# cherise215/advchain

Measured on AMD Instinct MI355X. Metric: augmented images/sec (N adv steps, chain=noise+bias+morph+affine), higher is better.
Workload: dtype f32

## Files before the change

advchain_amd/_lib.py:

```python
import ctypes
import os
from ctypes import c_char_p, c_float, c_int, c_int64, c_void_p

_HERE = os.path.dirname(os.path.abspath(__file__))
LIB_PATH = os.path.join(_HERE, "csrc", "libadvchain_hip.so")

_P, _I, _L, _F = c_void_p, c_int, c_int64, c_float

PROTOTYPES = {
    "advchain_version": (_I, []),
    "advchain_last_error": (c_char_p, []),
    "advchain_set_deterministic": (None, [_I]),
    "advchain_get_deterministic": (_I, []),
    "advchain_grid_sample_fwd": (_I, [_P, _P, _P, _L, _L, _I, _P, _P, _I, _I, _I, _P]),
    "advchain_grid_sample_fwd_ride": (_I, [_P, _P, _P, _P, _P, _L, _L, _I, _P, _P, _I, _I, _I, _I, _P]),
    "advchain_scatter_workspace": (_L, [_L, _I, _P]),
    "advchain_grid_sample_bwd": (_I, [_P, _P, _P, _P, _P, _P, _L, _L, _I, _P, _P, _I, _I, _I, _I, _P]),
    "advchain_window_stage_workspace": (_L, [_L, _L, _I, _P]),
    "advchain_grid_sample_bwd_staged": (_I, [_P, _P, _P, _P, _P, _P, _L, _L, _I, _P, _P, _I, _I, _I, _I, _P, _P]),
    "advchain_last_bwd_route": (_I, []),
    "advchain_det_warp_workspace": (_L, [_L, _L, _I, _P]),
    "advchain_grid_sample_bwd_det": (_I, [_P, _P, _P, _P, _P, _P, _L, _L, _I, _P, _P, _I, _I, _I, _P]),
    "advchain_compose_self_fwd": (_I, [_P, _P, _P, _L, _I, _P, _I, _P, _P]),
    "advchain_compose_self_bwd": (_I, [_P, _P, _P, _P, _I, _I, _L, _I, _P, _P]),
    "advchain_affine_warp_fwd": (_I, [_P, _P, _P, _L, _L, _I, _P, _I, _I, _P]),
    "advchain_affine_warp_fwd_ride": (_I, [_P, _P, _P, _P, _P, _L, _L, _I, _P, _I, _I, _I, _P]),
    "advchain_affine_warp_bwd_workspace": (_L, [_L, _I, _P]),
    "advchain_affine_warp_bwd": (_I, [_P, _P, _P, _P, _P, _P, _L, _L, _I, _P, _I, _I, _P]),
    "advchain_affine_warp_bwd_det": (_I, [_P, _P, _P, _P, _P, _P, _P, _L, _L, _I, _P, _I, _I, _P]),
    "advchain_affine_theta_fwd": (_I, [_P, _P, _F, _P, _P, _L, _I, _P]),
    "advchain_affine_theta_bwd": (_I, [_P, _P, _F, _P, _P, _P, _L, _I, _P]),
    "advchain_tp_interp_fwd": (_I, [_P, _P, _P, _P, _P, _P, _P, _L, _L, _I, _I, _F, _P, _P, _P]),
    "advchain_tp_interp_fwd_smoothed_pair": (_I, [_P, _P, _P, _P, _P, _P, _P, _P, _L, _L, _I, _F, _P, _P, _F, _P]),
    "advchain_band_reduce_axis": (_I, [_P, _P, _P, _P, _P, _P, _P, _P, _I, _L, _L, _F, _P]),
    "advchain_band_reduce_rows_dense": (_I, [_P, _P, _P, _P, _P, _L, _L, _L, _L, _F, _P]),
    "advchain_bias_field_fwd": (_I, [_P, _P, _P, _P, _P, _P, _P, _P, _P, _L, _L, _F, _I, _F, _P]),
    "advchain_bias_field_bwd": (_I, [_P, _P, _P, _P, _P, _P, _P, _P, _P, _P, _L, _L, _F, _I, _F, _P]),
    "advchain_bias_rows_per_wg": (_I, [_P, _L]),
    "advchain_bias_field_fwd_rows": (_I, [_P, _P, _P, _P, _P, _P, _P, _P, _P, _L, _L, _F, _I, _F, _I, _P]),
    "advchain_bias_field_bwd_rows": (_I, [_P, _P, _P, _P, _P, _P, _P, _P, _P, _P, _L, _L, _F, _I, _F, _I, _P]),
    "advchain_bias_field_bwd_reduced": (_I, [_P, _P, _P, _P, _P, _P, _P, _P, _P, _P, _L, _L, _F, _I, _F, _P, _P, _L, _I, _P]),
    "advchain_gauss_axis": (_I, [_P, _P, _P, _L, _L, _I, _P, _I, _P, _I, _I, _F, _P]),
    "advchain_gauss_axis_generic": (_I, [_P, _P, _L, _I, _P, _I, _P, _I, _F, _P]),
    "advchain_max_displacement": (_I, [_P, _P, _L, _I, _P, _P]),
    "advchain_grid_sample_bicubic2d_fwd": (_I, [_P, _P, _P, _L, _L, _P, _P, _I, _P]),
    "advchain_grid_sample_bicubic2d_bwd": (_I, [_P, _P, _P, _P, _P, _L, _L, _P, _P, _I, _P]),
    "advchain_affine_grid2d_fwd": (_I, [_P, _P, _L, _P, _P]),
    "advchain_affine_grid2d_bwd_workspace": (_L, [_L, _P]),
    "advchain_affine_grid2d_bwd": (_I, [_P, _P, _P, _L, _P, _P]),
    "advchain_slot_rows_max": (_I, [_P, _P, _L, _L, _I, _P]),
    "advchain_demons_compose_pair_fwd": (_I, [_P, _P, _P, _P, _P, _P, _P, _P, _P, _P, _P, _P, _P, _L, _I, _I, _P, _P, _F, _F, _I, _P]),
    "advchain_demons_compose_pair_bwd": (_I, [_P, _P, _P, _P, _P, _P, _P, _P, _P, _P, _P, _P, _P, _P, _P, _P, _P, _L, _P, _P, _P, _L,
                                              _I, _I, _P, _F, _F, _P]),
    "advchain_bounds_check": (_I, [_P, _P, _P, _L, _P, _P]),
    "advchain_expo_chain_fused_levels": (_I, [_L, _I, _P, _I, _P]),
    "advchain_expo_chain_fwd": (_I, [_P, _P, _P, _L, _I, _P, _I, _P, _P, _P, _P]),
    "advchain_expo_chain_bwd": (_I, [_P, _P, _P, _P, _P, _P, _P, _L, _I, _P, _I, _P]),
    "advchain_gauss_xy": (_I, [_P, _P, _P, _L, _L, _I, _P, _P, _I, _I, _F, _P, _P, _L]),
    "advchain_gauss_small": (_I, [_P, _P, _L, _I, _P, _P, _I, _F, _P]),
    "advchain_gauss_small_pair": (_I, [_P, _P, _L, _I, _P, _P, _F, _I, _P]),
    "advchain_axpy": (_I, [_P, _P, _P, _F, _L, _P]),
    "advchain_sign_axpy": (_I, [_P, _P, _P, _F, _L, _P, _P, _P]),
    "advchain_nonzero_mask": (_I, [_P, _P, _L, _P]),
    "advchain_consistency_finish": (_I, [_P, _P, _P, _P, _I, _P]),
    "advchain_norm_workspace": (_L, [_L, _L]),
    "advchain_norm_axpy": (_I, [_P, _P, _P, _P, _F, _L, _L, _P]),
    "advchain_norm_axpy_gated": (_I, [_P, _P, _P, _P, _F, _L, _L, _P, _P, _P]),
    "advchain_update_multi": (_I, [_P, _I, _P, _P]),
    "advchain_consistency_fwd": (_I, [_P, _P, _P, _P, _P, _P, _P, _L, _L, _I, _P, _I, _I, _I, _I, _P]),
    "advchain_consistency_bwd": (_I, [_P, _P, _P, _P, _P, _P, _F, _F, _F, _F, _I, _L, _L, _I, _P, _I, _P]),
    "advchain_consistency_fused_fwd": (_I, [_P, _P, _P, _P, _P, _L, _L, _I, _P, _I, _I, _I, _I, _P]),
    "advchain_consistency_fused_bwd": (_I, [_P, _P, _P, _P, _P, _P, _F, _F, _F, _F, _I, _L, _L, _I, _P, _I, _P]),
    "advchain_consistency_wide_fwd": (_I, [_P, _P, _P, _P, _P, _P, _L, _L, _I, _P, _I, _I, _I, _I, _P]),
    "advchain_consistency_wide_bwd": (_I, [_P, _P, _P, _P, _P, _P, _P, _F, _F, _F, _F, _I, _L, _L, _I, _P, _I, _P]),
    "advchain_consistency_ref_bwd": (_I, [_P, _P, _P, _P, _P, _P, _P, _F, _F, _F, _F, _I, _L, _L, _I, _P, _I, _P]),
    "advchain_set_ref_grad_reg_max_k": (None, [_I]),
    "advchain_get_ref_grad_reg_max_k": (_I, []),
    "advchain_consistency_lp_fwd": (_I, [_P, _I, _P, _I, _P, _P, _P, _P, _L, _L, _I, _P, _I, _I, _I, _I, _P]),
    "advchain_consistency_lp_bwd": (_I, [_P, _I, _P, _I, _P, _P, _P, _P, _P, _F, _F, _F, _F, _I, _L, _L, _I, _P, _I, _P]),
    "advchain_consistency_lp_ref_bwd": (_I, [_P, _I, _P, _I, _P, _P, _P, _P, _P, _F, _F, _F, _F, _I, _L, _L, _I, _P, _I, _P]),
    "advchain_consistency_cw_fwd": (_I, [_P, _I, _P, _I, _P, _P, _P, _P, _L, _L, _I, _P, _I, _I, _I, _I, _P, _P]),
    "advchain_consistency_cw_bwd": (_I, [_P, _I, _P, _I, _P, _P, _P, _P, _P, _F, _F, _F, _F, _I, _L, _L, _I, _P, _I, _P, _P]),
    "advchain_consistency_cw_ref_bwd": (_I, [_P, _I, _P, _I, _P, _P, _P, _P, _P, _F, _F, _F, _F, _I, _L, _L, _I, _P, _I, _P, _P]),
    "advchain_consistency_fused_fwd_bf16": (_I, [_P, _P, _P, _P, _P, _L, _L, _I, _P, _P]),
    "advchain_consistency_fused_bwd_bf16": (_I, [_P, _P, _P, _P, _P, _P, _F, _F, _F, _L, _L, _I, _P, _P]),
    "advchain_seg_loss_workspace": (_L, [_L, _I, _P]),
    "advchain_ce2d_fwd": (_I, [_P, _I, _P, _P, _P, _P, _P, _P, _L, _L, _P, _F, _P]),
    "advchain_ce2d_bwd": (_I, [_P, _I, _P, _P, _P, _P, _P, _P, _P, _L, _L, _P, _F, _P]),
    "advchain_contour_fwd": (_I, [_P, _P, _P, _P, _P, _P, _P, _L, _L, _I, _P, _I, _I, _P]),
    "advchain_contour_bwd": (_I, [_P, _P, _P, _P, _L, _L, _I, _P, _I, _P]),
    "advchain_one_hot": (_I, [_P, _P, _L, _L, _L, _P]),
    "advchain_dice_workspace": (_L, [_L, _L, _I, _P]),
    "advchain_dice_fwd": (_I, [_P, _I, _P, _P, _P, _P, _P, _P, _P, _L, _L, _I, _P, _I, _F, _F, _F, _P]),
    "advchain_dice_bwd": (_I, [_P, _I, _P, _P, _P, _P, _P, _P, _P, _P, _L, _L, _I, _P, _F, _F, _P]),
    "advchain_image_diff2d_fwd": (_I, [_P, _P, _P, _L, _L, _P, _P]),
    "advchain_image_diff2d_bwd": (_I, [_P, _P, _P, _L, _L, _P, _P]),
    "advchain_jacobian_det2d_fwd": (_I, [_P, _P, _L, _P, _P]),
    "advchain_jacobian_det2d_bwd": (_I, [_P, _P, _P, _L, _P, _P]),
    "advchain_expo_start": (_I, [_P, _P, _F, _L, _I, _P, _P]),
    "advchain_image_diff3d_fwd": (_I, [_P, _P, _P, _P, _L, _L, _P, _P]),
    "advchain_image_diff3d_bwd": (_I, [_P, _P, _P, _P, _L, _L, _P, _P]),
    "advchain_jacobian_det_fwd": (_I, [_P, _P, _L, _I, _P, _I, _P]),
    "advchain_jacobian_det_bwd": (_I, [_P, _P, _P, _P, _L, _I, _P, _I, _P]),
    "advchain_jacobian_det_workspace": (_L, [_L, _I, _P]),
    "advchain_jacobian_stats_workspace": (_L, [_L, _I, _P]),
    "advchain_jacobian_stats": (_I, [_P, _P, _P, _P, _P, _P, _L, _I, _P, _I, _P]),
    "advchain_sumsq_ordered": (_I, [_P, _L, _P, _P, _P]),
    "advchain_bicubic2d_det_workspace": (_L, [_L, _L, _P]),
    "advchain_grid_sample_bicubic2d_bwd_det": (_I, [_P, _P, _P, _P, _P, _P, _L, _L, _P, _P, _I, _P]),
    "advchain_tp_interp_sumsq_partials": (_L, [_P, _L]),
    "advchain_tp_interp_sumsq_ordered": (_I, [_P, _P, _P, _P, _P, _P, _L, _L, _P, _P, _P]),
# ... 109 lines not shown
```

advchain_amd/csrc/fields.hip:

```cpp
#include "sampler_common.h"

namespace advchain {

constexpr int kBandMax = 8;

struct BandAxis {
  const int* start;
  const float* w;
  const int* lo;
  const int* hi;
  int S, g, B;
};
struct BandTables { BandAxis a[3]; };

__device__ __forceinline__ void decode3(int v, const Dims& d, int& i0, int& i1, int& i2) {
  i2 = v % d.s2;
  const int r = v / d.s2;
  i1 = r % d.s1;
  i0 = r / d.s1;
}

__device__ __forceinline__ float tp_eval(const float* __restrict__ coef, const BandTables& T, int i0, int i1, int i2) {
  const BandAxis& A0 = T.a[0];
  const BandAxis& A1 = T.a[1];
// ... 961 lines not shown
    float t[4] = {v.x, v.y, v.z, v.w};
#pragma unroll
    for (int o = 0; o < 4; ++o) {
      if (PRE == 1) t[o] *= scale;
      if (PRE == 2) {
        float sl;
        t[o] = border_identity(t[o], Sc, sl) - lin_coord(caxis == 2 ? 4 * q + o : (caxis == 1 ? gy : iz), Sc);
      }
      if (!inr) t[o] = 0.f;
    }
    *reinterpret_cast<float4*>(A + r * PA + 4 + 4 * q) = make_float4(t[0], t[1], t[2], t[3]);
  }
  __syncthreads();
  for (int e = threadIdx.x; e < R * Q; e += kBlock) {
    const int r = e / Q, q = e - r * Q;
    const float* a = A + r * PA + 4 * q;
    const float4 a0 = *reinterpret_cast<const float4*>(a), a1 = *reinterpret_cast<const float4*>(a + 4),
                 a2 = *reinterpret_cast<const float4*>(a + 8);
    const float win[12] = {a0.x, a0.y, a0.z, a0.w, a1.x, a1.y, a1.z, a1.w, a2.x, a2.y, a2.z, a2.w};
    float acc[4] = {0.f, 0.f, 0.f, 0.f};
#pragma unroll
    for (int o = 0; o < 4; ++o)
#pragma unroll
      for (int k = 0; k < 9; ++k) acc[o] += gw.w[k] * win[o + k];
    *reinterpret_cast<float4*>(B + r * W + 4 * q) = make_float4(acc[0], acc[1], acc[2], acc[3]);
  }
  __syncthreads();
  for (int e = threadIdx.x; e < TY * Q; e += kBlock) {
    const int ry = e / Q, q = e - ry * Q;
    const int gy = y0 + ry;
    if (gy >= d.s1) continue;
    float acc[4] = {0.f, 0.f, 0.f, 0.f};
#pragma unroll
    for (int k = 0; k < 9; ++k) {
      const float4 b = *reinterpret_cast<const float4*>(B + (ry + k) * W + 4 * q);
      acc[0] += gw.w[k] * b.x; acc[1] += gw.w[k] * b.y; acc[2] += gw.w[k] * b.z; acc[3] += gw.w[k] * b.w;
    }
    const int64_t off = base + (int64_t)gy * W + 4 * q;
    if (POST == 1) {
#pragma unroll
      for (int o = 0; o < 4; ++o) acc[o] += lin_coord(caxis == 2 ? 4 * q + o : (caxis == 1 ? gy : iz), Sc);
    }
    if (POST == 2) {
      const float4 a4 = *reinterpret_cast<const float4*>(aux + off);
      const float av[4] = {a4.x, a4.y, a4.z, a4.w};
#pragma unroll
      for (int o = 0; o < 4; ++o) {
        float slope;
        border_identity(av[o], Sc, slope);
        acc[o] *= slope;
      }
    }
    *reinterpret_cast<float4*>(out + off) = make_float4(acc[0], acc[1], acc[2], acc[3]);
  }
}

constexpr int kGaussMarchU = 9;
template <int PRE, int POST>
__global__ void __launch_bounds__(kBlock)
k_gauss_march_z(const float* __restrict__ in, float* __restrict__ out, const float* __restrict__ aux, int64_t planes, Dims d,
                int C, GaussW gw, float scale, int zc, int nchunk) {
  constexpr int U = kGaussMarchU;
  const int q = d.s2 >> 2;
  int64_t r = (int64_t)blockIdx.x * kBlock + threadIdx.x;
  const int xq = (int)(r % q);
  r /= q;
  const int iy = (int)(r % d.s1);
  r /= d.s1;
  const int chunk = (int)(r % nchunk);
  const int64_t plane = r / nchunk;
  if (plane >= planes) return;
  const int V = (int)d.voxels();
  const int stride = d.s1 * d.s2;
  const int caxis = 2 - (int)(plane % C);
  const int Sc = caxis == 2 ? d.s2 : (caxis == 1 ? d.s1 : d.s0);
  const int ix = xq * 4;
  const float* src = in + plane * V + iy * d.s2 + ix;
  float* dst = out + plane * V + iy * d.s2 + ix;
  const float* ax = POST == 2 ? aux + plane * V + iy * d.s2 + ix : nullptr;
  auto fetch = [&](int j) -> float4 {
    return *reinterpret_cast<const float4*>(src + (int64_t)min(max(j, 0), d.s0 - 1) * stride);
  };
  auto prep = [&](float4 v, int j) -> float4 {
    if (j < 0 || j >= d.s0) return make_float4(0.f, 0.f, 0.f, 0.f);
    if (PRE == 1) return make_float4(v.x * scale, v.y * scale, v.z * scale, v.w * scale);
    if (PRE == 2) {
      float sl;
      float e[4] = {v.x, v.y, v.z, v.w};
#pragma unroll
      for (int o = 0; o < 4; ++o) e[o] = border_identity(e[o], Sc, sl) - lin_coord(caxis == 2 ? ix + o : (caxis == 1 ? iy : j), Sc);
      return make_float4(e[0], e[1], e[2], e[3]);
    }
    return v;
  };
  const int ja = chunk * zc, jb = min(ja + zc, d.s0);
  float4 w[8 + U];
#pragma unroll
  for (int k = 0; k < 8; ++k) w[k] = prep(fetch(ja - 4 + k), ja - 4 + k);
  for (int j0 = ja; j0 < jb; j0 += U) {
    float4 nw[U];
#pragma unroll
    for (int u = 0; u < U; ++u) nw[u] = fetch(j0 + 4 + u);
#pragma unroll
    for (int u = 0; u < U; ++u) w[8 + u] = prep(nw[u], j0 + 4 + u);
#pragma unroll
    for (int u = 0; u < U; ++u) {
// ... 665 lines not shown
    dim3 gm(advchain_blocks(threads, kBlock));
#define GM(PRE, POST) hipLaunchKernelGGL((k_gauss_march_z<PRE, POST>), gm, blk, 0, st, in, out, aux, planes, d, (int)C, gw, scale, zc, nchunk)
    switch (pre * 3 + post) {
      case 0: GM(0, 0); break;
      case 1: GM(0, 1); break;
      case 2: GM(0, 2); break;
      case 3: GM(1, 0); break;
      case 4: GM(1, 1); break;
      case 5: GM(1, 2); break;
      case 6: GM(2, 0); break;
      case 7: GM(2, 1); break;
      default: GM(2, 2); break;
    }
#undef GM
    ADVCHAIN_LAUNCH_CHECK();
    return ADVCHAIN_OK;
  }
#define GA(PRE, POST)                                                                                                     \
  do {                                                                                                                    \
    if (!v4) hipLaunchKernelGGL((k_gauss_axis<PRE, POST>), grid, blk, 0, st, in, out, aux, total, d, (int)C, axis, gw, scale); \
    else if (axis == 2) hipLaunchKernelGGL((k_gauss_axis_v4<PRE, POST, 2>), grid, blk, 0, st, in, out, aux, total / 4, d, (int)C, gw, scale, riw); \
    else if (axis == 1) hipLaunchKernelGGL((k_gauss_axis_v4<PRE, POST, 1>), grid, blk, 0, st, in, out, aux, total / 4, d, (int)C, gw, scale, 0); \
    else hipLaunchKernelGGL((k_gauss_axis_v4<PRE, POST, 0>), grid, blk, 0, st, in, out, aux, total / 4, d, (int)C, gw, scale, 0); \
  } while (0)
  switch (pre * 3 + post) {
    case 0: GA(0, 0); break;
    case 1: GA(0, 1); break;
    case 2: GA(0, 2); break;
    case 3: GA(1, 0); break;
    case 4: GA(1, 1); break;
    case 5: GA(1, 2); break;
    case 6: GA(2, 0); break;
    case 7: GA(2, 1); break;
    default: GA(2, 2); break;
  }
#undef GA
  ADVCHAIN_LAUNCH_CHECK();
  return ADVCHAIN_OK;
}

}

bool advchain_gauss_xy_takes(int ndim, const int64_t* dims, int64_t planes) {
  static const bool off = getenv("ADVCHAIN_NO_GAUSS_XY") != nullptr;
  if (off || !fdims_ok(ndim, dims)) return false;
  const Dims d = fmake_dims(ndim, dims);
  if ((d.s2 & 3) != 0 || d.s2 < 8 || d.s2 > 512 || d.s1 < 8 || planes > 65535 || d.s0 > 65535) return false;
  int TY = 32;
  while (TY > 8 && (size_t)(TY + 8) * (2 * d.s2 + 8) * 4 > 53248) TY >>= 1;
  if (TY > d.s1) TY = (d.s1 + 7) / 8 * 8;
  return (size_t)(TY + 8) * (2 * d.s2 + 8) * sizeof(float) <= 65536;
}

extern "C" {

int advchain_gauss_xy(const float* in, float* out, const float* aux, int64_t planes, int64_t C, int ndim, const int64_t* dims,
                      const float* weights9, int pre, int post, float scale, void* stream, const float* in_hi, int64_t planes_lo) {
  ADVCHAIN_CHECK_ARG(in && out && in != out && weights9, "gauss_xy: null/aliased pointer");
  ADVCHAIN_CHECK_ARG(fdims_ok(ndim, dims), "gauss_xy: bad dims");
  ADVCHAIN_CHECK_ARG(C >= 1 && C <= 3 && pre >= 0 && pre <= 2 && post >= 0 && post <= 2 && (post != 2 || aux), "gauss_xy: bad C/pre/post");
  ADVCHAIN_CHECK_ARG(post == 0 || ndim == 2, "gauss_xy: post belongs to the last axis");
  const Dims d = fmake_dims(ndim, dims);
  static const bool off = getenv("ADVCHAIN_NO_GAUSS_XY") != nullptr;
  if (off || (d.s2 & 3) != 0 || d.s2 < 8 || d.s2 > 512 || d.s1 < 8 || planes > 65535 || d.s0 > 65535 ||
      ((reinterpret_cast<uintptr_t>(in) | reinterpret_cast<uintptr_t>(out) | reinterpret_cast<uintptr_t>(aux) |
        reinterpret_cast<uintptr_t>(in_hi)) & 15) != 0)
    return ADVCHAIN_ERR_UNSUPPORTED;
  ADVCHAIN_CHECK_ARG(!in_hi || (planes_lo > 0 && planes_lo < planes), "gauss_xy: bad split of the input planes");
  if (planes == 0 || d.voxels() == 0) return ADVCHAIN_OK;
  int TY = 32;
  while (TY > 8 && (size_t)(TY + 8) * (2 * d.s2 + 8) * 4 > 53248) TY >>= 1;
  if (TY > d.s1) TY = (d.s1 + 7) / 8 * 8;
  const size_t lds = (size_t)(TY + 8) * (2 * d.s2 + 8) * sizeof(float);
  if (lds > 65536) return ADVCHAIN_ERR_UNSUPPORTED;
  GaussW gw;
  for (int k = 0; k < 9; ++k) gw.w[k] = weights9[k];
  dim3 grid((unsigned)((d.s1 + TY - 1) / TY), (unsigned)d.s0, (unsigned)planes);
  hipStream_t st = (hipStream_t)stream;
#define GXY(PRE, POST) hipLaunchKernelGGL((k_gauss_xy<PRE, POST>), grid, dim3(kBlock), lds, st, in, out, aux, d, (int)C, gw, scale, TY, in_hi, (int)planes_lo)
  switch (pre * 3 + post) {
    case 0: GXY(0, 0); break;
    case 1: GXY(0, 1); break;
    case 2: GXY(0, 2); break;
    case 3: GXY(1, 0); break;
    case 4: GXY(1, 1); break;
    case 5: GXY(1, 2); break;
    case 6: GXY(2, 0); break;
    case 7: GXY(2, 1); break;
    default: GXY(2, 2); break;
  }
#undef GXY
  ADVCHAIN_LAUNCH_CHECK();
  return ADVCHAIN_OK;
}

static int gauss_small_launch(const float* in, float* out, int64_t planes, int ndim, const int64_t* dims,
                              const float* weights9, int pre, float scale, int mirror, void* stream) {
  ADVCHAIN_CHECK_ARG(in && out && in != out && weights9, "gauss_small: null/aliased pointer");
  ADVCHAIN_CHECK_ARG(fdims_ok(ndim, dims), "gauss_small: bad dims");
  ADVCHAIN_CHECK_ARG(pre == 0 || pre == 1, "gauss_small: pre must be 0 or 1");
  const Dims d = fmake_dims(ndim, dims);
  ADVCHAIN_CHECK_ARG(d.voxels() <= kGaussSmallMax, "gauss_small: plane larger than 4096 voxels");
  ADVCHAIN_CHECK_ARG(planes >= 0 && planes < (1ll << 30), "gauss_small: bad plane count");
  if (planes == 0) return ADVCHAIN_OK;
  GaussW gw;
  for (int k = 0; k < 9; ++k) gw.w[k] = weights9[k];
  const unsigned blocks = (unsigned)(mirror == 1 ? 2 * planes : planes);
  if (d.voxels() > 1024)
    hipLaunchKernelGGL(k_gauss_small<1024>, dim3(blocks), dim3(1024), 0, (hipStream_t)stream, in, out, d, ndim, gw,
                       pre == 1 ? scale : 1.f, mirror, (int)planes);
  else
    hipLaunchKernelGGL(k_gauss_small<kBlock>, dim3(blocks), dim3(kBlock), 0, (hipStream_t)stream, in, out, d, ndim, gw,
                       pre == 1 ? scale : 1.f, mirror, (int)planes);
  ADVCHAIN_LAUNCH_CHECK();
  return ADVCHAIN_OK;
}

int advchain_gauss_small(const float* in, float* out, int64_t planes, int ndim, const int64_t* dims,
                         const float* weights9, int pre, float scale, void* stream) {
  return gauss_small_launch(in, out, planes, ndim, dims, weights9, pre, scale, 0, stream);
}

int advchain_gauss_small_pair(const float* in, float* out, int64_t planes, int ndim, const int64_t* dims,
                              const float* weights9, float scale, int adjoint, void* stream) {
  return gauss_small_launch(in, out, planes, ndim, dims, weights9, 1, scale, adjoint ? 2 : 1, stream);
}

int advchain_sign_axpy(const float* base, const float* x, float* out, float a, int64_t n, const float* gate, const float* old,
                       void* stream) {
  ADVCHAIN_CHECK_ARG(x && out && n >= 0 && (!gate || old), "sign_axpy: null pointer");
  if (n == 0) return ADVCHAIN_OK;
// ... 76 lines not shown
```

advchain_amd/ops.py:

```python
import collections
import ctypes
import functools
import os

import numpy as np
import torch

from . import _lib
from .bands import gaussian_weights_1d

_INTERP = {"bilinear": 0, "trilinear": 0, "linear": 0, "nearest": 1, "bicubic": 2}
_PAD = {"zeros": 0, "border": 1, "reflection": 2}
_GAUSS9 = _lib.float_array(gaussian_weights_1d(1.0))
_GAUSS9_CACHE = {}


GENERIC_MAX_TAPS = 129


def gauss9(sigma, taps=None):
    sigma = float(sigma)
    if taps is None:
        taps = 2 * int(4 * sigma + 0.5) + 1
    taps = int(taps)
# ... 91 lines not shown
    return _PAD[padding_mode]


def _hint_bits(disp):
    if disp is None or not disp == disp or disp < 0:
        return 0
    return min(int(disp) + 1, 255) << 8


def _fine_bits(disp):
    if disp is None or not disp == disp or disp < 0:
        return 0
    return max(1, min(int(disp * 1024.0) + 1, (1 << 22) - 1))


def raw_grid_sample_fwd(inp, grid, interp, padding, clamp_grid, disp_hint=None):
    N, C = inp.shape[:2]
    nd = inp.dim() - 2
    odims = grid.shape[2:]
    out = torch.empty((N, C) + tuple(odims), device=inp.device, dtype=torch.float32)
    _lib.check(_lib.load().advchain_grid_sample_fwd(_ptr(inp), _ptr(grid), _ptr(out), N, C, nd,
                                                    _lib.dims_array(inp.shape[2:]), _lib.dims_array(odims),
                                                    interp, padding, int(clamp_grid) | _hint_bits(disp_hint), _stream()),
               "grid_sample_fwd")
    return out


def raw_grid_sample_fwd_ride(inp, grid, ride, interp, padding, clamp_grid, nonzero, disp_hint=None):
    N, C = inp.shape[:2]
    nd = inp.dim() - 2
    odims = tuple(grid.shape[2:])
    out = torch.empty((N, C) + odims, device=inp.device, dtype=torch.float32)
    rout = torch.empty((N, 1) + odims, device=inp.device, dtype=torch.float32)
    _lib.check(_lib.load().advchain_grid_sample_fwd_ride(_ptr(inp), _ptr(grid), _ptr(out), _ptr(ride), _ptr(rout), N, C, nd,
                                                         _lib.dims_array(inp.shape[2:]), _lib.dims_array(odims), interp, padding,
                                                         int(clamp_grid) | _hint_bits(disp_hint), int(bool(nonzero)), _stream()),
               "grid_sample_fwd_ride")
    return out, rout


DISP_SLOTS = 4096
ADAPTIVE_HALO = os.environ.get("ADVCHAIN_NO_ADAPTIVE_HALO") is None
PAIR_FIELDS = os.environ.get("ADVCHAIN_NO_PAIR_FIELDS") is None
TILED_SCATTER = True
FUSED_LOSS = True
WIDE_LOSS_MIN_K = 17
REF_GRAD_REG_MAX_K = 4
FUSE_2D = True
COMPOSITE = True
RIDE_MASK = True
RIDE_INTERPS = ("bilinear", "trilinear", "linear", "nearest")
WINDOW_STAGED = True
WINDOW_STAGED_CHANNELS = (1, 2, 4)
BIAS_REDUCED = True

BWD_ROUTES = ("none", "general", "rows", "gather", "march", "window_float", "window_int64", "window_staged", "tiled")


def last_bwd_route():
    return BWD_ROUTES[_lib.load().advchain_last_bwd_route()]


def set_deterministic(on):
    _lib.load().advchain_set_deterministic(1 if on else 0)


def is_deterministic():
    return bool(_lib.load().advchain_get_deterministic())


def _scatter_workspace(N, dims, device):
    n = _lib.load().advchain_scatter_workspace(N, len(dims), _lib.dims_array(dims))
    return torch.empty(n, device=device, dtype=torch.int32)


def _det_warp_workspace(N, C, dims, device):
    n = _lib.load().advchain_det_warp_workspace(N, C, len(dims), _lib.dims_array(dims))
    return torch.empty(max(1, n), device=device, dtype=torch.int32)


def _general_warp_kernel(C, interp, in_dims, out_dims):
    return C > 4 or interp != 0 or tuple(in_dims) != tuple(out_dims)


def raw_grid_sample_bwd(gout, inp, grid, interp, padding, clamp_grid, need_gin, need_ggrid, halo=0):
    N, C = inp.shape[:2]
    nd = inp.dim() - 2
    if need_gin and is_deterministic() and _general_warp_kernel(C, interp, inp.shape[2:], grid.shape[2:]):
        ws = _det_warp_workspace(N, C, inp.shape[2:], inp.device)
        gin = torch.empty_like(inp)
        ggrid = torch.empty_like(grid) if need_ggrid else None
        _lib.check(_lib.load().advchain_grid_sample_bwd_det(_ptr(gout), _ptr(inp), _ptr(grid), _ptr(gin), _ptr(ggrid), _ptr(ws),
                                                            N, C, nd, _lib.dims_array(inp.shape[2:]),
                                                            _lib.dims_array(grid.shape[2:]), interp, padding, int(clamp_grid),
                                                            _stream()), "grid_sample_bwd_det")
        return gin, ggrid
    tiled = TILED_SCATTER and need_gin
    ws = _scatter_workspace(N, inp.shape[2:], inp.device) if tiled else None
    gin = (torch.empty_like(inp) if tiled else torch.zeros_like(inp)) if need_gin else None
    ggrid = torch.empty_like(grid) if need_ggrid else None
    if (tiled and WINDOW_STAGED and nd == 2 and C in WINDOW_STAGED_CHANNELS and is_deterministic()
            and not _general_warp_kernel(C, interp, inp.shape[2:], grid.shape[2:])):
        lib = _lib.load()
        n = lib.advchain_window_stage_workspace(N, C, nd, _lib.dims_array(inp.shape[2:]))
        stage = torch.empty(max(4, n), device=inp.device, dtype=torch.int32)
        _lib.check(lib.advchain_grid_sample_bwd_staged(_ptr(gout), _ptr(inp), _ptr(grid), _ptr(gin), _ptr(ggrid), _ptr(ws),
# ... 160 lines not shown
        return _halo_3d(disp)
    if 16 - 0.001 <= disp < 32 - 0.001:
        return -24 if disp < 24 - 0.001 else -32
    return _halo_2d(disp)


def _halo_3d(disp):
    for h in (2, 3, 4):
        if disp < h - 0.001:
            return -h
    return 8


def _halo_2d(disp):
    for h in (2, 3, 4, 6, 8, 12, 16):
        if disp < h - 0.001:
            return -h
    return 16


def raw_gauss(x, C, pre=0, post=0, scale=1.0, aux=None, weights=None):
    w9 = weights or _GAUSS9
    x_hi = None
    if isinstance(x, (tuple, list)):
        x, x_hi = x
        shape = (x.shape[0] + x_hi.shape[0],) + tuple(x.shape[1:])
    else:
        shape = tuple(x.shape)
    nd = x.dim() - 2
    planes = shape[0] * shape[1]
    dims = _lib.dims_array(x.shape[2:])
    axes = [2, 1, 0][:nd]
    lib = _lib.load()
    if len(w9) != 9:
        if post != 0 or pre not in (0, 1):
            raise NotImplementedError("the fused prologue / epilogue of the Gaussian exists for the 9-tap window only")
        cur = torch.cat([x, x_hi], 0) if x_hi is not None else x
        cur = cur if cur.is_contiguous() else cur.contiguous()
        for i, ax in enumerate(axes):
            out = torch.empty_like(cur)
            _lib.check(lib.advchain_gauss_axis_generic(_ptr(cur), _ptr(out), planes, nd, dims, ax, w9, len(w9),
                                                       float(scale) if (pre == 1 and i == 0) else 1.0, _stream()),
                       "gauss_axis_generic")
            cur = out
        return cur
    if x_hi is not None and (x[0, 0].numel() <= 4096 or not (x.is_contiguous() and x_hi.is_contiguous())):
        x, x_hi = torch.cat([x, x_hi], 0), None
    if post == 0 and pre in (0, 1) and x[0, 0].numel() <= 4096:
        out = torch.empty_like(x)
        _lib.check(lib.advchain_gauss_small(_ptr(x), _ptr(out), planes, nd, dims, w9, pre, float(scale), _stream()),
                   "gauss_small")
        return out
    cur = x
    out = torch.empty(shape, device=x.device, dtype=torch.float32)
    rc = lib.advchain_gauss_xy(_ptr(x), _ptr(out), _ptr(aux) if (post == 2 and nd == 2) else None, planes, C, nd, dims, w9,
                               pre, post if nd == 2 else 0, float(scale) if pre == 1 else 1.0, _stream(), _ptr(x_hi),
                               x.shape[0] * x.shape[1])
    if rc == 0:
        if nd == 2:
            return out
        out2 = torch.empty_like(out)
        _lib.check(lib.advchain_gauss_axis(_ptr(out), _ptr(out2), _ptr(aux) if post == 2 else None, planes, C, nd, dims, 0,
                                           w9, 0, post, 1.0, _stream()), "gauss_axis")
        return out2
    if rc != -2:
        _lib.check(rc, "gauss_xy")
    if x_hi is not None:
        x = cur = torch.cat([x, x_hi], 0)
    for i, ax in enumerate(axes):
        out = torch.empty_like(x)
        p = pre if i == 0 else 0
        q = post if i == len(axes) - 1 else 0
        _lib.check(lib.advchain_gauss_axis(_ptr(cur), _ptr(out), _ptr(aux) if q == 2 else None, planes, C, nd, dims, ax,
                                           w9, p, q, float(scale) if p == 1 else 1.0, _stream()), "gauss_axis")
        cur = out
    return cur


def raw_tp_interp(coef, tables, C, add_identity=False, scale=1.0, want_out=True, sumsq=None, disp_out=None, out=None):
    planes = coef.shape[0] * coef.shape[1]
    if want_out and out is None:
        out = torch.empty((coef.shape[0], coef.shape[1]) + tuple(tables.full_dims), device=coef.device,
                          dtype=torch.float32)
    _lib.check(_lib.load().advchain_tp_interp_fwd(_ptr(coef), _ptr(out), _ptr(tables.itab), _ptr(tables.ftab),
                                                  _lib.dims_array(tables.S), _lib.dims_array(tables.g),
                                                  _lib.dims_array(tables.B), planes, C, tables.ndim,
                                                  int(add_identity), float(scale), _ptr(sumsq), _ptr(disp_out),
                                                  _stream()),
               "tp_interp_fwd")
    return out


def field_sumsq(coef, tables, C):
    coef = _dev(coef, "coefficients")
    if is_deterministic():
        lib = _lib.load()
        planes = coef.shape[0] * coef.shape[1]
        S = _lib.dims_array(tables.S)
        partials = torch.empty(max(1, lib.advchain_tp_interp_sumsq_partials(S, planes)), device=coef.device, dtype=torch.float32)
        out = torch.empty(1, device=coef.device, dtype=torch.float32)
        _lib.check(lib.advchain_tp_interp_sumsq_ordered(_ptr(coef), _ptr(tables.itab), _ptr(tables.ftab), S,
                                                        _lib.dims_array(tables.g), _lib.dims_array(tables.B), planes, C,
                                                        _ptr(partials), _ptr(out), _stream()), "tp_interp_sumsq_ordered")
        return out
    slots = torch.zeros(64, device=coef.device, dtype=torch.float32)
    raw_tp_interp(coef, tables, C, want_out=False, sumsq=slots)
# ... 711 lines not shown
        while True:
            out = _DemonsField._enqueue_chain(ctx, vel, s1, tables, d, n, scale, w9, pos_only, composite, plan, frozen, pair)
            if norm_rb is None:
                break
            norm, want = float(norm_rb.values()[0]), int(n_base)
            while norm / (2.0 ** want) > 0.5:
                want += 1
            norm_rb = None
            _NSTEPS_HINT[nkey] = want
            NSTEPS_STATS["chains"] += 1
            if plan is not None:
                if want != n:
                    del plan.pending[mark:]
                plan.pending.insert(mark, ("nsteps", dict(n=want, n_base=int(n_base))))
            if want == n:
                break
            NSTEPS_STATS["respeculated"] += 1
            n = want
        return out

    @staticmethod
    def _enqueue_chain(ctx, vel, s1, tables, d, n, scale, w9, pos_only, composite, plan, frozen, pair):
        N = s1.shape[0]
        inv = 1.0 / (2.0 ** n)
        disp = _persistent_zeros("disp", (n + 2, DISP_SLOTS), vel.device) if ADAPTIVE_HALO else None
        row = (lambda m: None) if disp is None else (lambda m: disp[m])
        key = (str(s1.device), tuple(s1.shape), n, HINT_SLOT)
        site = None
        if frozen:
            if disp is None:
                raise PlanMismatch("launch plan: a frozen chain needs the measured displacements (ADVCHAIN_NO_ADAPTIVE_HALO is set)")
            site = plan.take("chain", n=n, d=d)
            hints = site["bounds"].values()
        else:
            pend = _PENDING_BOUNDS.pop(key, None)
            if pend is not None and pend.event.query():
                _note_chain_bounds(key, pend.values(), n)
            hints = _CHAIN_HINTS.get(key)
        full = (N, d) + tuple(tables.full_dims)
        phi0 = torch.empty(full, device=vel.device, dtype=torch.float32) if composite else \
            raw_tp_interp(s1, tables, d, add_identity=True, scale=inv, disp_out=row(0))
        fields = torch.empty((n - 1,) + tuple(phi0.shape), device=phi0.device, dtype=torch.float32)
        pos = torch.empty_like(phi0)
        harr = None if hints is None else (ctypes.c_int32 * n)(*[(_hint_bits(hints[m]) >> 8) | (_fine_bits(hints[m]) << 8)
                                                                 for m in range(n)])
        if COUNT_FUSED and harr is not None and disp is not None and FUSE_2D:
            FUSE_STATS["fused_levels"] += _lib.load().advchain_expo_chain_fused_levels(phi0.shape[0], d, _lib.dims_array(phi0.shape[2:]), n, harr)
        try:
            rows_max = rc = None
            if composite:
                q = torch.empty_like(phi0)
                rows_max = None if disp is None else (plan.slot(site) if site is not None else
                                                      torch.empty(disp.shape[0], device=vel.device, dtype=torch.float32))
                rc = _lib.load().advchain_demons_compose_pair_fwd(
                    _ptr(vel), _ptr(s1), _ptr(phi0), _ptr(fields), _ptr(pos), _ptr(q), _ptr(disp), _ptr(rows_max), _ptr(tables.itab),
                    _ptr(tables.ftab), _lib.dims_array(tables.S), _lib.dims_array(tables.g), _lib.dims_array(tables.B),
                    vel.shape[0], d, n, harr, w9, float(scale), float(inv), int(bool(FUSE_2D)), _stream())
                if rc == -2:
                    composite = ctx.composite = False
                    raw_gauss_small_pair_into(vel, s1, scale, w9)
                    raw_tp_interp(s1, tables, d, add_identity=True, scale=inv, disp_out=row(0), out=phi0)
                else:
                    _lib.check(rc, "demons_compose_pair_fwd")
            if not composite:
                _lib.check(_lib.load().advchain_expo_chain_fwd(_ptr(phi0), _ptr(fields), _ptr(pos), phi0.shape[0], d,
                                                               _lib.dims_array(phi0.shape[2:]), n, _ptr(disp), harr,
                                                               None if (disp is None or not FUSE_2D) else _ptr(disp[n + 1]), _stream()),
                           "expo_chain_fwd")
                q = pos if pos_only else raw_gauss(pos, d, pre=2, post=1, weights=w9)
                rows_max = None if disp is None else raw_slot_rows_max(disp, reset=True, out=None if site is None else plan.slot(site))
        except BaseException:
            if disp is not None:
                _forget_persistent(disp)
            raise
        ctx.save_for_backward(pos, phi0, fields)
        ctx.frozen = site is not None
        if site is not None:
            plan.check(rows_max, site)
            ctx.disp = site["bounds"]
        else:
            ctx.disp = None if rows_max is None else _Readback(rows_max)
            if ctx.disp is not None:
                _PENDING_BOUNDS[key] = ctx.disp
                if plan is not None:
                    plan.note("chain", rb=ctx.disp, n=n, d=d)
        global _LAST_FIELD_BOUND
        _LAST_FIELD_BOUND = None if ctx.disp is None else (ctx.disp, n)
        ctx.cfg = (scale, tables, inv, d)
        ctx.nsteps = n
        ctx.hint_key = key
        if pair:
            return q[:N // 2], q[N // 2:]
        return q

    @staticmethod
    def backward(ctx, *grads):
        pos, phi0, fields = ctx.saved_tensors
        scale, tables, inv, d = ctx.cfg
        smooth_iter, w9, pos_only = ctx.opts
        gq = tuple(_dev(g, "grad") for g in grads) if ctx.pair else _dev(grads[0], "grad")
        composite = (ctx.composite and TILED_SCATTER and ctx.pair and gq[0].is_contiguous() and gq[1].is_contiguous()
                     and gq[0].shape == gq[1].shape)
        if composite:
            gpos = torch.empty_like(pos)
        elif pos_only:
            gpos = torch.cat(gq, 0) if ctx.pair else gq.contiguous()
        else:
            gpos = raw_gauss(gq, d, post=2, aux=pos, weights=w9)
        g = gpos
        ws = _scatter_workspace(gpos.shape[0], gpos.shape[2:], gpos.device) if TILED_SCATTER else None
        n = ctx.nsteps
        if ctx.disp is not None:
            dm = ctx.disp.values()
            if not ctx.frozen:
                _PENDING_BOUNDS.pop(ctx.hint_key, None)
                _note_chain_bounds(ctx.hint_key, dm, n)
            halos = [squaring_halo(dm[m], d) for m in range(n - 1, -1, -1)]
        else:
            big = 2 if d == 3 else 16
            halos = [big, big, max(1, big // 2)] + [1 if d == 3 else 2] * n
        halos = halos[:n]
        if composite:
            N2 = gpos.shape[0]
            S, gg = list(tables.S), list(tables.g)
            g, scratch = torch.empty_like(gpos), torch.empty_like(gpos)
            t1 = torch.empty((N2, d, S[1], gg[2]), device=gpos.device, dtype=torch.float32)
            gs1 = torch.empty((N2, d, gg[1], gg[2]), device=gpos.device, dtype=torch.float32)
            gvel = torch.empty((N2 // 2, d, gg[1], gg[2]), device=gpos.device, dtype=torch.float32)
            wd, wlo, WB = tables.dense_inner
            rc = _lib.load().advchain_demons_compose_pair_bwd(
                _ptr(gq[0]), _ptr(gq[1]), _ptr(pos), _ptr(phi0), _ptr(fields), _ptr(gpos), _ptr(g), _ptr(scratch), _ptr(ws), _ptr(t1),
                _ptr(gs1), _ptr(gvel), (ctypes.c_int32 * n)(*[int(h) for h in halos]), _ptr(tables.itab), _ptr(tables.ftab), _ptr(wd),
                _ptr(wlo), int(WB), _lib.dims_array(S), _lib.dims_array(gg), _lib.dims_array(tables.B), N2 // 2, d, n, w9, float(scale),
                float(inv), _stream())
            if rc != -2:
                _lib.check(rc, "demons_compose_pair_bwd")
                return gvel, None, None, None, None, None, None
            gpos = raw_gauss(gq, d, post=2, aux=pos, weights=w9)
            g = gpos
        if ws is None:
            phis = [phi0] + list(fields.unbind(0))
            for i, phi in enumerate(reversed(phis)):
                g = raw_compose_self_bwd(g, phi, None, chain=False, halo=halos[i])
        else:
            g, scratch = torch.empty_like(gpos), torch.empty_like(gpos)
            _lib.check(_lib.load().advchain_expo_chain_bwd(_ptr(gpos), _ptr(phi0), _ptr(fields), _ptr(g), _ptr(scratch), _ptr(ws),
                                                           (ctypes.c_int32 * n)(*[int(h) for h in halos]), gpos.shape[0], d,
                                                           _lib.dims_array(gpos.shape[2:]), n, _stream()), "expo_chain_bwd")
        gs1 = raw_tp_adjoint(g, tables, gfull2=gpos, scale=inv)
        for _ in range(smooth_iter - 1):
            gs1 = raw_gauss(gs1, d, weights=w9)
        gvel = raw_gauss_small_pair(gs1, scale, adjoint=True, weights=w9) if ctx.pair else None
        if gvel is None:
            gvel = raw_gauss(gs1, d, pre=1, scale=scale, weights=w9)
            if ctx.pair:
                h = gvel.shape[0] // 2
                gvel = gvel[:h] - gvel[h:]
        return gvel, None, None, None, None, None, None


_LAST_FIELD_BOUND = None
HINT_SLOT = 0
FUSE_STATS = {"chains": 0, "refused": 0, "fused_levels": 0}
COUNT_FUSED = False


class _HintCache(dict):
    CAP = 256

    def __setitem__(self, key, value):
        if len(self) >= self.CAP and key not in self:
            self.clear()
        dict.__setitem__(self, key, value)


_NSTEPS_HINT = _HintCache()
NSTEPS_STATS = {"chains": 0, "respeculated": 0}
_PENDING_BOUNDS = _HintCache()


def _note_chain_bounds(key, dm, n):
    FUSE_STATS["chains"] += 1
# ... 845 lines not shown
```

include/advchain_hip.h:

```cpp
#ifndef ADVCHAIN_HIP_H_
#define ADVCHAIN_HIP_H_

#include <stdint.h>

#ifdef __cplusplus
extern "C" {
#endif

#define ADVCHAIN_INTERP_LINEAR 0
#define ADVCHAIN_INTERP_NEAREST 1
#define ADVCHAIN_INTERP_BICUBIC 2
#define ADVCHAIN_PAD_ZEROS 0
#define ADVCHAIN_PAD_BORDER 1
#define ADVCHAIN_PAD_REFLECTION 2

int advchain_version(void);
const char* advchain_last_error(void);

void advchain_set_deterministic(int on);
int advchain_get_deterministic(void);

int advchain_grid_sample_fwd(const float* in, const float* grid, float* out, int64_t N, int64_t C, int ndim,
                             const int64_t* in_dims, const int64_t* out_dims, int interp, int padding,
                             int clamp_grid, void* stream);
// ... 80 lines not shown
                               void* stream);

int advchain_affine_theta_fwd(const float* param, const float* cfg_host, float param_scale, float* theta,
                              float* theta_inv, int64_t N, int ndim, void* stream);
int advchain_affine_theta_bwd(const float* param, const float* cfg_host, float param_scale, const float* grad_theta,
                              const float* grad_theta_inv, float* grad_param, int64_t N, int ndim, void* stream);

int advchain_tp_interp_fwd(const float* coef, float* out, const int32_t* itab, const float* ftab, const int64_t* S,
                           const int64_t* g, const int64_t* B, int64_t planes, int64_t C, int ndim, int add_identity,
                           float scale, float* sumsq, float* disp_out, void* stream);
int64_t advchain_tp_interp_sumsq_partials(const int64_t* S, int64_t planes);
int advchain_tp_interp_sumsq_ordered(const float* coef, const int32_t* itab, const float* ftab, const int64_t* S, const int64_t* g,
                                     const int64_t* B, int64_t planes, int64_t C, float* partials, float* out, void* stream);
int advchain_tp_interp_fwd_smoothed_pair(const float* vel, float* s1, float* out, const int32_t* itab, const float* ftab,
                                         const int64_t* S, const int64_t* g, const int64_t* B, int64_t P, int64_t C,
                                         int add_identity, float scale, float* disp_out, const float* weights9, float gscale,
                                         void* stream);
int advchain_band_reduce_axis(const float* in, const float* in2, float* out, const int32_t* itab, const float* ftab,
                              const int64_t* S, const int64_t* g, const int64_t* B, int axis, int64_t outer,
                              int64_t inner, float scale, void* stream);
int advchain_band_reduce_rows_dense(const float* in, const float* in2, float* out, const float* wd, const int32_t* lo,
                                    int64_t rows, int64_t S, int64_t g, int64_t WB, float scale, void* stream);

int advchain_bias_field_fwd(const float* cp, const float* data, float* out, float* field, const int32_t* itab,
                            const float* ftab, const int64_t* S, const int64_t* g, const int64_t* B, int64_t N,
                            int64_t C, float eps, int use_log, float cp_scale, void* stream);
int advchain_bias_field_bwd(const float* cp, const float* data, const float* grad_out, float* grad_L, float* grad_data,
                            const int32_t* itab, const float* ftab, const int64_t* S, const int64_t* g,
                            const int64_t* B, int64_t N, int64_t C, float eps, int use_log, float cp_scale,
                            void* stream);
int advchain_bias_rows_per_wg(const int64_t* S, int64_t N);
int advchain_bias_field_fwd_rows(const float* cp, const float* data, float* out, float* field, const int32_t* itab,
                                 const float* ftab, const int64_t* S, const int64_t* g, const int64_t* B, int64_t N,
                                 int64_t C, float eps, int use_log, float cp_scale, int rows_per_wg, void* stream);
int advchain_bias_field_bwd_rows(const float* cp, const float* data, const float* grad_out, float* grad_L, float* grad_data,
                                 const int32_t* itab, const float* ftab, const int64_t* S, const int64_t* g,
                                 const int64_t* B, int64_t N, int64_t C, float eps, int use_log, float cp_scale,
                                 int rows_per_wg, void* stream);
int advchain_bias_field_bwd_reduced(const float* cp, const float* data, const float* grad_out, float* t1, float* grad_data,
                                    const int32_t* itab, const float* ftab, const int64_t* S, const int64_t* g,
                                    const int64_t* B, int64_t N, int64_t C, float eps, int use_log, float cp_scale,
                                    const float* wd, const int32_t* lo, int64_t WB, int rows_per_wg, void* stream);

int advchain_gauss_axis(const float* in, float* out, const float* aux, int64_t planes, int64_t C, int ndim,
                        const int64_t* dims, int axis, const float* weights9_host, int pre, int post, float scale,
                        void* stream);

int advchain_gauss_axis_generic(const float* in, float* out, int64_t planes, int ndim, const int64_t* dims, int axis,
                                const float* weights_host, int ntaps, float scale, void* stream);

int advchain_gauss_xy(const float* in, float* out, const float* aux, int64_t planes, int64_t C, int ndim, const int64_t* dims,
                      const float* weights9, int pre, int post, float scale, void* stream, const float* in_hi,
                      int64_t planes_lo);
int advchain_gauss_small(const float* in, float* out, int64_t planes, int ndim, const int64_t* dims,
                         const float* weights9_host, int pre, float scale, void* stream);

int advchain_gauss_small_pair(const float* in, float* out, int64_t planes, int ndim, const int64_t* dims,
                              const float* weights9_host, float scale, int adjoint, void* stream);

int advchain_axpy(const float* x, const float* y, float* out, float a, int64_t n, void* stream);
int advchain_sign_axpy(const float* base, const float* x, float* out, float a, int64_t n, const float* gate, const float* old,
                       void* stream);
int advchain_nonzero_mask(const float* x, float* out, int64_t n, void* stream);
int64_t advchain_norm_workspace(int64_t N, int64_t M);
int advchain_norm_axpy(const float* base, const float* x, float* out, float* workspace, float step, int64_t N,
                       int64_t M, void* stream);
int advchain_norm_axpy_gated(const float* base, const float* x, float* out, float* workspace, float step, int64_t N,
                             int64_t M, const float* gate, const float* old, void* stream);
typedef struct advchain_update_desc {
  const float* base;
  const float* x;
  float* out;
  const float* old;
  int64_t N;
  int64_t M;
  int32_t kind;
  float step;
} advchain_update_desc;
int advchain_update_multi(const advchain_update_desc* descs, int n, const float* gate, void* stream);

int advchain_consistency_fwd(const float* pred, const float* ref, const float* mask, float* P, float* D, float* R,
                             float* sums, int64_t N, int64_t K, int ndim, const int64_t* dims, int mask_channels,
                             int ref_is_prob, int want_edges, int want_kl, void* stream);
int advchain_consistency_finish(float* slots, const float* coef4_host, float* sums, float* value, int reset, void* stream);
int advchain_consistency_bwd(const float* P, const float* D, const float* R, const float* mask,
                             const float* grad_scale, float* grad_pred, float c_mse, float c_a, float c_b, float c_kl,
                             int kl_is_gt, int64_t N, int64_t K, int ndim, const int64_t* dims, int mask_channels,
                             void* stream);
int advchain_consistency_fused_fwd(const float* pred, const float* ref, const float* mask, float* R, float* sums, int64_t N,
                                   int64_t K, int ndim, const int64_t* dims, int mask_channels, int ref_is_prob, int want_edges,
                                   int want_kl, void* stream);
int advchain_consistency_fused_bwd(const float* pred, const float* ref, const float* R, const float* mask,
                                   const float* grad_scale, float* grad_pred, float c_mse, float c_a, float c_b, float c_kl,
                                   int ref_is_prob, int64_t N, int64_t K, int ndim, const int64_t* dims, int mask_channels,
                                   void* stream);

int advchain_consistency_wide_fwd(const float* pred, const float* ref, const float* mask, float* stats, float* R, float* sums,
                                  int64_t N, int64_t K, int ndim, const int64_t* dims, int mask_channels, int ref_is_prob,
                                  int want_edges, int want_kl, void* stream);
int advchain_consistency_wide_bwd(const float* pred, const float* ref, const float* stats, const float* R, const float* mask,
                                  const float* grad_scale, float* grad_pred, float c_mse, float c_a, float c_b, float c_kl,
                                  int ref_is_prob, int64_t N, int64_t K, int ndim, const int64_t* dims, int mask_channels,
                                  void* stream);

int advchain_consistency_ref_bwd(const float* pred, const float* ref, const float* stats ,
                                 const float* R , const float* mask, const float* grad_scale,
// ... 112 lines not shown
```

Measured before the change: 4411.

## Add register-marching wave-level separable gauss_xy kernel for 2D fields

Adds a k_gauss_xy_march kernel that gives each wavefront group a strip of rows. It does the x-direction 9-tap pass with lane shuffles and keeps a sliding window of x-filtered rows in registers for the y pass, so no LDS tile is needed. With the default form setting, the new kernel is chosen when the input is 2D (s0==1), pre!=2 and the width is at most 256. The march length is picked so that enough waves are launched. The aim is to avoid LDS staging and block-level sync overhead in the 2D Gaussian smoothing used by the morph/demons path. The cost is more register pressure and redundant halo row loads per strip.

```diff
diff --git a/advchain_amd/_lib.py b/advchain_amd/_lib.py
--- a/advchain_amd/_lib.py
+++ b/advchain_amd/_lib.py
@@ -57,6 +57,8 @@
     "advchain_expo_chain_fwd": (_I, [_P, _P, _P, _L, _I, _P, _I, _P, _P, _P, _P]),
     "advchain_expo_chain_bwd": (_I, [_P, _P, _P, _P, _P, _P, _P, _L, _I, _P, _I, _P]),
     "advchain_gauss_xy": (_I, [_P, _P, _P, _L, _L, _I, _P, _P, _I, _I, _F, _P, _P, _L]),
+    "advchain_set_gauss_xy_form": (None, [_I]),
+    "advchain_gauss_xy_form_for": (_I, [_I, _P, _L, _I]),
     "advchain_gauss_small": (_I, [_P, _P, _L, _I, _P, _P, _I, _F, _P]),
     "advchain_gauss_small_pair": (_I, [_P, _P, _L, _I, _P, _P, _F, _I, _P]),
     "advchain_axpy": (_I, [_P, _P, _P, _F, _L, _P]),
diff --git a/advchain_amd/csrc/fields.hip b/advchain_amd/csrc/fields.hip
--- a/advchain_amd/csrc/fields.hip
+++ b/advchain_amd/csrc/fields.hip
@@ -1037,6 +1037,140 @@
       }
     }
     *reinterpret_cast<float4*>(out + off) = make_float4(acc[0], acc[1], acc[2], acc[3]);
+  }
+}
+
+__device__ __forceinline__ float lin_coord_sel(int i, int S) {
+  const float step = 2.f / (float)(S - 1);
+  const float v = (i < S / 2) ? __builtin_fmaf(step, (float)i, -1.f) : __builtin_fmaf(-step, (float)(S - 1 - i), 1.f);
+  return S <= 1 ? (S == 1 ? -1.f : 0.f) : v;
+}
+__device__ __forceinline__ float border_identity_sel(float pos, int S, float& slope) {
+  const float sm1 = (float)(S - 1);
+  const float xu = ((pos + 1.f) * 0.5f) * sm1;
+  const bool lo = xu <= 0.f, hi = xu >= sm1;
+  const float x = lo ? 0.f : (hi ? sm1 : xu);
+  const float mult = (lo || hi) ? 0.f : 0.5f * sm1;
+  const float f = floorf(x);
+  const int i0 = (int)f;
+  const int i1 = min(i0 + 1, S - 1);
+  const float a = lin_coord_sel(i0, S), b = lin_coord_sel(i1, S);
+  slope = mult * (b - a);
+  return __builtin_fmaf((f + 1.f) - x, a, (x - f) * b);
+}
+template <bool B> struct GaussXYFlag { static constexpr bool value = B; };
+template <int PRE, int POST>
+__global__ void __launch_bounds__(kBlock)
+k_gauss_xy_march(const float* __restrict__ in, float* __restrict__ out, const float* __restrict__ aux, Dims d, int C, GaussW gw,
+                 float scale, int mlen, const float* __restrict__ in_hi, int planes_lo, int planes) {
+  const int W = d.s2, H = d.s1;
+  const int lpr = W >> 2, gpw = 64 / lpr;
+  const int lane = threadIdx.x & 63;
+  const int grp = lane / lpr, xq = lane - grp * lpr;
+  const int ny = (H + mlen - 1) / mlen, spp = d.s0 * ny;
+  const int wpp = (spp + gpw - 1) / gpw;
+  const unsigned wave = blockIdx.x * (kBlock / 64) + __builtin_amdgcn_readfirstlane((int)(threadIdx.x >> 6));
+  const int plane = (int)(wave / (unsigned)wpp);
+  if (plane >= planes) return;
+  const int sidx = (int)(wave - (unsigned)plane * wpp) * gpw + grp;
+  if (grp >= gpw || sidx >= spp) return;
+  const int iz = sidx / ny;
+  const int y0 = min((sidx - iz * ny) * mlen, H - mlen);
+  const int x = 4 * xq;
+  const bool first = xq == 0, last = xq == lpr - 1;
+  const int caxis = 2 - plane % C;
+  const int Sc = caxis == 2 ? d.s2 : (caxis == 1 ? d.s1 : d.s0);
+  const int64_t base = ((int64_t)plane * d.s0 + iz) * H * (int64_t)W + x;
+  const float* src = (in_hi && plane >= planes_lo) ? in_hi + (((int64_t)(plane - planes_lo) * d.s0 + iz) * H * (int64_t)W + x) : in + base;
+  const float* ax = POST == 2 ? aux + base : nullptr;
+  float* dst = out + base;
+  auto fetch = [&](const float* p, int r) -> float4 {
+    return *reinterpret_cast<const float4*>(p + (int64_t)min(max(r, 0), H - 1) * W);
+  };
+  auto xrow = [&](float4 v, int gy) -> float4 {
+    const bool inr = gy >= 0 && gy < H;
+    float t[4] = {v.x, v.y, v.z, v.w};
+#pragma unroll
+    for (int o = 0; o < 4; ++o) {
+      if (PRE == 1) t[o] *= scale;
+      if (PRE == 2) {
+        float sl;
+        t[o] = border_identity_sel(t[o], Sc, sl) - lin_coord_sel(caxis == 2 ? x + o : (caxis == 1 ? gy : iz), Sc);
+      }
+      if (!inr) t[o] = 0.f;
+    }
+    float win[12];
+#pragma unroll
+    for (int k = 0; k < 4; ++k) {
+      const float pv = lane_prev_f(t[k]), nx = lane_next_f(t[k]);
+      win[k] = first ? 0.f : pv;
+      win[4 + k] = t[k];
+      win[8 + k] = last ? 0.f : nx;
+    }
+    float acc[4] = {0.f, 0.f, 0.f, 0.f};
+#pragma unroll
+    for (int o = 0; o < 4; ++o)
+#pragma unroll
+      for (int k = 0; k < 9; ++k) acc[o] = __builtin_fmaf(gw.w[k], win[o + k], acc[o]);
+    return make_float4(acc[0], acc[1], acc[2], acc[3]);
+  };
+  constexpr int R = PRE == 2 ? 4 : 8;
+  float4 xw[8 + R];
+  float4 raw[R], axr[POST == 2 ? R : 1];
+  {
+    float4 head[8];
+#pragma unroll
+    for (int u = 0; u < 8; ++u) head[u] = fetch(src, y0 - 4 + u);
+#pragma unroll
+    for (int u = 0; u < R; ++u) raw[u] = fetch(src, y0 + 4 + u);
+    if (POST == 2) {
+#pragma unroll
+      for (int u = 0; u < R; ++u) axr[u] = fetch(ax, y0 + u);
+    }
+#pragma unroll
+    for (int u = 0; u < 8; ++u) xw[u] = xrow(head[u], y0 - 4 + u);
+  }
+  auto round = [&](int j0, auto more) {
+#pragma unroll
+    for (int u = 0; u < R; ++u) {
+      const int j = j0 + u;
+      xw[8 + u] = xrow(raw[u], j + 4);
+      if (decltype(more)::value) raw[u] = fetch(src, j + 4 + R);
+      float acc[4] = {0.f, 0.f, 0.f, 0.f};
+#pragma unroll
+      for (int k = 0; k < 9; ++k) {
+        const float4 b = xw[u + k];
+        acc[0] = __builtin_fmaf(gw.w[k], b.x, acc[0]);
+        acc[1] = __builtin_fmaf(gw.w[k], b.y, acc[1]);
+        acc[2] = __builtin_fmaf(gw.w[k], b.z, acc[2]);
+        acc[3] = __builtin_fmaf(gw.w[k], b.w, acc[3]);
+      }
+      if (POST == 1) {
+#pragma unroll
+        for (int o = 0; o < 4; ++o) acc[o] += lin_coord_sel(caxis == 2 ? x + o : (caxis == 1 ? j : iz), Sc);
+      }
+      if (POST == 2) {
+        const float4 a4 = axr[u];
+        if (decltype(more)::value) axr[u] = fetch(ax, j + R);
+        const float av[4] = {a4.x, a4.y, a4.z, a4.w};
+#pragma unroll
+        for (int o = 0; o < 4; ++o) {
+          float slope;
+          border_identity_sel(av[o], Sc, slope);
+          acc[o] *= slope;
+        }
+      }
+      *reinterpret_cast<float4*>(dst + (int64_t)j * W) = make_float4(acc[0], acc[1], acc[2], acc[3]);
+    }
+#pragma unroll
+    for (int k = 0; k < 8; ++k) xw[k] = xw[R + k];
+  };
+  if (PRE == 2) {
+    for (int j0 = y0; j0 < y0 + mlen; j0 += R) round(j0, GaussXYFlag<true>{});
+  } else {
+    const int jl = y0 + mlen - R;
+    for (int j0 = y0; j0 < jl; j0 += R) round(j0, GaussXYFlag<true>{});
+    round(jl, GaussXYFlag<false>{});
   }
 }
 
@@ -1808,7 +1942,33 @@
   return (size_t)(TY + 8) * (2 * d.s2 + 8) * sizeof(float) <= 65536;
 }
 
+static int g_gauss_xy_form = 0;
+
+static inline bool gauss_xy_march_takes(const Dims& d) { return (d.s2 & 3) == 0 && d.s2 >= 8 && d.s2 <= 256 && d.s1 >= 8; }
+
+static inline int64_t gauss_xy_march_waves(const Dims& d, int64_t planes, int m) {
+  const int64_t gpw = 64 / (d.s2 / 4), spp = (int64_t)d.s0 * ((d.s1 + m - 1) / m);
+  return planes * ((spp + gpw - 1) / gpw);
+}
+static inline int gauss_xy_march_len(const Dims& d, int64_t planes) {
+  for (int m = 32; m > 8; m /= 2)
+    if (m <= d.s1 && gauss_xy_march_waves(d, planes, m) >= 1024) return m;
+  return 8;
+}
+
+static inline int gauss_xy_form_of(const Dims& d, int64_t planes, int pre) {
+  if (!gauss_xy_march_takes(d) || g_gauss_xy_form == 1 || gauss_xy_march_waves(d, planes, 8) >= (1ll << 31)) return 1;
+  return (g_gauss_xy_form == 2 || (pre != 2 && d.s0 == 1)) ? 2 : 1;
+}
+
 extern "C" {
+
+void advchain_set_gauss_xy_form(int form) { g_gauss_xy_form = (form >= 0 && form <= 2) ? form : 0; }
+
+int advchain_gauss_xy_form_for(int ndim, const int64_t* dims, int64_t planes, int pre) {
+  if (!dims || !advchain_gauss_xy_takes(ndim, dims, planes)) return 0;
+  return gauss_xy_form_of(fmake_dims(ndim, dims), planes, pre);
+}
 
 int advchain_gauss_xy(const float* in, float* out, const float* aux, int64_t planes, int64_t C, int ndim, const int64_t* dims,
                       const float* weights9, int pre, int post, float scale, void* stream, const float* in_hi, int64_t planes_lo) {
@@ -1831,8 +1991,27 @@
   if (lds > 65536) return ADVCHAIN_ERR_UNSUPPORTED;
   GaussW gw;
   for (int k = 0; k < 9; ++k) gw.w[k] = weights9[k];
+  hipStream_t st = (hipStream_t)stream;
+  if (gauss_xy_form_of(d, planes, pre) == 2) {
+    const int mlen = gauss_xy_march_len(d, planes);
+    dim3 gm((unsigned)((gauss_xy_march_waves(d, planes, mlen) + kBlock / 64 - 1) / (kBlock / 64)));
+#define GXM(PRE, POST) hipLaunchKernelGGL((k_gauss_xy_march<PRE, POST>), gm, dim3(kBlock), 0, st, in, out, aux, d, (int)C, gw, scale, mlen, in_hi, (int)planes_lo, (int)planes)
+    switch (pre * 3 + post) {
+      case 0: GXM(0, 0); break;
+      case 1: GXM(0, 1); break;
+      case 2: GXM(0, 2); break;
+      case 3: GXM(1, 0); break;
+      case 4: GXM(1, 1); break;
+      case 5: GXM(1, 2); break;
+      case 6: GXM(2, 0); break;
+      case 7: GXM(2, 1); break;
+      default: GXM(2, 2); break;
+    }
+#undef GXM
+    ADVCHAIN_LAUNCH_CHECK();
+    return ADVCHAIN_OK;
+  }
   dim3 grid((unsigned)((d.s1 + TY - 1) / TY), (unsigned)d.s0, (unsigned)planes);
-  hipStream_t st = (hipStream_t)stream;
 #define GXY(PRE, POST) hipLaunchKernelGGL((k_gauss_xy<PRE, POST>), grid, dim3(kBlock), lds, st, in, out, aux, d, (int)C, gw, scale, TY, in_hi, (int)planes_lo)
   switch (pre * 3 + post) {
     case 0: GXY(0, 0); break;
diff --git a/advchain_amd/ops.py b/advchain_amd/ops.py
--- a/advchain_amd/ops.py
+++ b/advchain_amd/ops.py
@@ -167,6 +167,7 @@
 RIDE_INTERPS = ("bilinear", "trilinear", "linear", "nearest")
 WINDOW_STAGED = True
 WINDOW_STAGED_CHANNELS = (1, 2, 4)
+GAUSS_XY_FORM = 0
 BIAS_REDUCED = True
 
 BWD_ROUTES = ("none", "general", "rows", "gather", "march", "window_float", "window_int64", "window_staged", "tiled")
@@ -433,6 +434,7 @@
                    "gauss_small")
         return out
     cur = x
+    lib.advchain_set_gauss_xy_form(int(GAUSS_XY_FORM))
     out = torch.empty(shape, device=x.device, dtype=torch.float32)
     rc = lib.advchain_gauss_xy(_ptr(x), _ptr(out), _ptr(aux) if (post == 2 and nd == 2) else None, planes, C, nd, dims, w9,
                                pre, post if nd == 2 else 0, float(scale) if pre == 1 else 1.0, _stream(), _ptr(x_hi),
@@ -1250,6 +1252,7 @@
                 q = torch.empty_like(phi0)
                 rows_max = None if disp is None else (plan.slot(site) if site is not None else
                                                       torch.empty(disp.shape[0], device=vel.device, dtype=torch.float32))
+                _lib.load().advchain_set_gauss_xy_form(int(GAUSS_XY_FORM))
                 rc = _lib.load().advchain_demons_compose_pair_fwd(
                     _ptr(vel), _ptr(s1), _ptr(phi0), _ptr(fields), _ptr(pos), _ptr(q), _ptr(disp), _ptr(rows_max), _ptr(tables.itab),
                     _ptr(tables.ftab), _lib.dims_array(tables.S), _lib.dims_array(tables.g), _lib.dims_array(tables.B),
@@ -1326,6 +1329,7 @@
             gs1 = torch.empty((N2, d, gg[1], gg[2]), device=gpos.device, dtype=torch.float32)
             gvel = torch.empty((N2 // 2, d, gg[1], gg[2]), device=gpos.device, dtype=torch.float32)
             wd, wlo, WB = tables.dense_inner
+            _lib.load().advchain_set_gauss_xy_form(int(GAUSS_XY_FORM))
             rc = _lib.load().advchain_demons_compose_pair_bwd(
                 _ptr(gq[0]), _ptr(gq[1]), _ptr(pos), _ptr(phi0), _ptr(fields), _ptr(gpos), _ptr(g), _ptr(scratch), _ptr(ws), _ptr(t1),
                 _ptr(gs1), _ptr(gvel), (ctypes.c_int32 * n)(*[int(h) for h in halos]), _ptr(tables.itab), _ptr(tables.ftab), _ptr(wd),
diff --git a/include/advchain_hip.h b/include/advchain_hip.h
--- a/include/advchain_hip.h
+++ b/include/advchain_hip.h
@@ -156,6 +156,8 @@
 int advchain_gauss_xy(const float* in, float* out, const float* aux, int64_t planes, int64_t C, int ndim, const int64_t* dims,
                       const float* weights9, int pre, int post, float scale, void* stream, const float* in_hi,
                       int64_t planes_lo);
+void advchain_set_gauss_xy_form(int form);
+int advchain_gauss_xy_form_for(int ndim, const int64_t* dims, int64_t planes, int pre);
 int advchain_gauss_small(const float* in, float* out, int64_t planes, int ndim, const int64_t* dims,
                          const float* weights9_host, int pre, float scale, void* stream);
 
```

New measurement: 4392. Within noise of the previous version (-0.4%).
